# dpfried/action-segmentation

Measured on AMD Instinct MI355X. Metric: frames/sec semi-Markov decode, CrossTask T~10k K~20 L=1024, 1/2/4/8 GPUs, higher is better.
Workload: dtype f64

## Files before the change

### action-segmentation_amd/csrc/smm_api.hip

```cpp
#include <algorithm>
#include <atomic>
#include <functional>
#include <cstdio>
#include <cstdlib>
#include <cstring>
#include <numeric>
#include <vector>
#include <unordered_map>
#include <mutex>
#include <utility>
#include <string>

#include "../../include/smmdp.h"
#include "smm_device.h"
#include "smm_launch.h"
#include "smm_plan_feedback.h"

static thread_local int g_last_hip = 0;

namespace {
struct SmmEnv {
    int spec = 1;
    int no_split = 0;
    double split_min_us = 100.0, split_ns = 0.0;
// ... 225 lines not shown
    for (int i = 0; i < s->b; ++i)
        if (lengths[i] < 1 || lengths[i] > s->t_max) return false;
    return true;
}

struct Carver {
    size_t cur;
    size_t packed(size_t bytes) { const size_t o = cur; cur += bytes; return o; }
    size_t take(size_t bytes) { const size_t o = packed(bytes); cur = align_up(cur, 256); return o; }
};

static void plan_meta(const smm_shape *s, SmmPlan *p)
{
    Carver c{0};
    c.take(sizeof(SmmVideo) * s->b);
    p->o_order = c.take(sizeof(int32_t) * s->b);
    p->o_nstates = c.take(sizeof(int32_t) * s->n_groups);
    p->o_emcum = c.take(sizeof(int32_t) * ((size_t)s->b + 1));
    p->o_err = c.cur;
    p->meta_bytes = p->o_err + 512;
}

static SmmPlan make_plan(const smm_shape *s, const int64_t *lengths)
{
    SmmPlan p{};
    p.b = (size_t)s->b;
    plan_meta(s, &p);
    size_t h = 0;
    for (int i = 0; i < s->b; ++i) h += 8 * (size_t)s->c_max * (size_t)(lengths[i] + 1);
    p.hist_doubles = h;
    p.elp_doubles = (size_t)s->total_frames * s->c_max;
    p.tab_doubles = (size_t)s->n_groups * s->c_max * ((size_t)s->c_max + 1 + s->k_rows) + (size_t)s->b * s->c_max;
    p.band_doubles = (size_t)s->n_groups * s->c_max * ((size_t)SMM_BAND_ROW + SMM_BAND_TAB + 64);
    {
        const size_t um = chunk_units_max(s);
        p.chunk_bytes = align_up(sizeof(int32_t) * s->b, 256) + align_up(sizeof(double) * um * s->c_max, 256) +
                        chunk_ext_meta_bytes(s->b, um, s->b);
    }
    p.o_chunk = align_up(p.meta_bytes + 8 * (p.hist_doubles + p.elp_doubles + p.tab_doubles + p.band_doubles), 256);
    p.total = p.o_chunk + p.chunk_bytes + 1024;
    return p;
}

extern "C" size_t smm_workspace_bytes(const smm_shape *shape, const int64_t *lengths_host)
{
    if (!shape_ok(shape) || !lengths_host || !lengths_ok(shape, lengths_host)) return 0;
    return make_plan(shape, lengths_host).total;
}

extern "C" size_t smm_error_word_offset(const smm_shape *shape)
{
    if (!shape_ok(shape)) return 0;
    SmmPlan p{};
    plan_meta(shape, &p);
    return p.o_err;
}

struct Staged {
    SmmVideo *videos;
    int32_t *order;
    int32_t *n_states;
    int32_t *err;
    double *hist;
    double *elp;
    double *tabs;
    double *band;
    bool band_mode;
    int32_t *em_cum;
    std::vector<int32_t> em_cum_host;
    int em_tpw, em_blocks;
    int kp_max, c_need;
    int n_split;
    SmmVideo *uvideos;
    int32_t *uorder, *porder;
    SmmChunkVideo *cvs;
    int32_t *redo;
    double *anchors;
    int n_cv, n_units, u_part1;
    int small_first, small_count;
    uint64_t *stamps = nullptr;
    hipEvent_t done = nullptr;
    void *fb_entry = nullptr;
    std::vector<int32_t> order_host, frames_host;
};

static bool band_mode(int kp_max, int c_need);

static int device_cus()
{
    static std::mutex mu;
    static int n_cu[64] = {};
    int dev = 0;
    if (hipGetDevice(&dev) != hipSuccess || dev < 0 || dev >= 64) return 0;
    std::lock_guard<std::mutex> lock(mu);
    if (!n_cu[dev] && hipDeviceGetAttribute(&n_cu[dev], hipDeviceAttributeMultiprocessorCount, dev) != hipSuccess) n_cu[dev] = 0;
    return n_cu[dev] > 0 ? n_cu[dev] : 0;
}

constexpr double SMM_BAND_NS_BASE = 145.0, SMM_BAND_NS_PER_STATE = 2.0;
extern "C" double smm_band_frame_ns(int n_states)
{
    if (n_states < 1 || n_states > SMM_MAX_STATES) return 0.0;
    return SMM_BAND_NS_BASE + SMM_BAND_NS_PER_STATE * n_states;
}

static double dp_frame_ns(bool band, int c) { return band ? smm_band_frame_ns(c) : 150.0 + 3.0 * c; }

static int choose_split(const SmmVideo *hv, int32_t *order, int b, int d, int c_max, int64_t total_frames)
{
    const SmmEnv &ev = env();
    if (b < 24 || ev.no_split) return 0;
    const int n_cu = device_cus();
    if (n_cu <= 0) return 0;
    const double em_us = (double)total_frames * (4.0 * d + 8.0 * c_max) / 4.0e6;
    if (em_us < ev.split_min_us) return 0;
    int tmax = 0;
    for (int i = 0; i < b; ++i) tmax = std::max(tmax, hv[i].T);
    const double split_ns = ev.split_ns > 0.0 ? ev.split_ns : 1.75 * smm_band_frame_ns(std::min(c_max, (int)SMM_MAX_STATES));
    const int thr = tmax - (int)(em_us * 1000.0 / split_ns) - ev.split_margin;
    int n1 = 0;
    for (int i = 0; i < b; ++i) n1 += hv[i].T >= thr;
    if (thr <= 0 || n1 < 1 || n1 > b / 3 || n1 > n_cu / 2 || b - n1 < 16 || b > 2 * n_cu) return 0;
    std::stable_partition(order, order + b, [&](int32_t v) { return hv[v].T >= thr; });
    return n1;
}

namespace {
struct PlanFeedback {
    uint64_t *stamps = nullptr;
    hipEvent_t done = nullptr;
    bool pending = false;
    bool have = false;
    bool busy = false;
    int evals_left = 5, n_replans = 0;
    int b = 0, n1_first = 0;
    double em_us = 0.0, end_before_us = 0.0, end_after_us = 0.0;
    std::vector<uint64_t> snap, used;
    std::vector<int32_t> order, frames;
};
constexpr int SMM_FEEDBACK_MAX_REPLANS = 4;
constexpr double SMM_FEEDBACK_MIN_GAIN = 0.02;
struct PlanEntry {
    PlanFeedback *fb = nullptr;
    std::vector<char> key;
    int device = 0;
    char *dev_meta = nullptr;
    SmmPlan plan{};
    Staged st{};
    hipEvent_t ready = nullptr;
    hipStream_t stream = nullptr;
    bool settled = false;
};
struct PlanSlabs {
    char *cur = nullptr;
    size_t left = 0;
    std::vector<std::pair<char *, size_t>> all;
};
struct PlanCache {
    std::mutex mu;
    std::unordered_map<uint64_t, std::vector<PlanEntry *>> entries;
    std::unordered_map<uint64_t, uint32_t> seen_once;
    size_t n = 0, bytes = 0, key_bytes = 0;
    size_t pinned_bytes = 0;
    uint64_t generation = 1;
    PlanSlabs slabs[64];
} g_plans;
// ... 11 lines not shown
    if (dev < 0 || dev >= 64) return nullptr;
    PlanSlabs &sl = g_plans.slabs[dev];
    bytes = align_up(bytes, 256);
    if (bytes > sl.left) {
        const size_t want = std::max(bytes, SMM_PLAN_SLAB);
        char *p = nullptr;
        if (hipMalloc(reinterpret_cast<void **>(&p), want) != hipSuccess) { (void)hipGetLastError(); return nullptr; }
        sl.all.emplace_back(p, want);
        sl.cur = p;
        sl.left = want;
    }
    char *r = sl.cur;
    sl.cur += bytes;
    sl.left -= bytes;
    return r;
}

void plan_key_append(std::vector<char> &k, const void *p, size_t n)
{
    const char *c = static_cast<const char *>(p);
    k.insert(k.end(), c, c + n);
}

std::vector<char> plan_key(const smm_shape *s, const int64_t *lengths, const int64_t *frame_off, const int32_t *group,
                           const int32_t *kp, const int32_t *n_states, bool for_viterbi, int cum_chunk, bool want_split)
{
    std::vector<char> k;
    k.reserve(sizeof(*s) + (size_t)s->b * 24 + (size_t)s->n_groups * 4 + 128);
    plan_key_append(k, s, sizeof(*s));
    plan_key_append(k, lengths, sizeof(int64_t) * s->b);
    plan_key_append(k, frame_off, sizeof(int64_t) * s->b);
    const char has[2] = {(char)(group != nullptr), (char)(kp != nullptr)};
    plan_key_append(k, has, 2);
    if (group) plan_key_append(k, group, sizeof(int32_t) * s->b);
    if (kp) plan_key_append(k, kp, sizeof(int32_t) * s->b);
    plan_key_append(k, n_states, sizeof(int32_t) * s->n_groups);
    const int32_t f[3] = {for_viterbi, cum_chunk, want_split};
    plan_key_append(k, f, sizeof(f));
    const std::string &ek = env().key;
    plan_key_append(k, ek.data(), ek.size() + 1);
    return k;
}

void feedback_arm(PlanEntry *e, Staged *out)
{
    PlanFeedback *fb = e->fb;
    if (!fb || !env().plan_feedback) return;
    out->fb_entry = e;
    if (fb->pending) {
        if (hipEventQuery(fb->done) != hipSuccess) { (void)hipGetLastError(); return; }
        fb->pending = false;
        bool complete = !fb->have && !fb->busy;
        for (int i = 0; complete && i < fb->b; ++i) complete = fb->stamps[2 * i] > 0 && fb->stamps[2 * i + 1] >= fb->stamps[2 * i];
        if (complete) { fb->snap.assign(fb->stamps, fb->stamps + 2 * (size_t)fb->b); fb->have = true; }
    }
    if (fb->evals_left > 0 && !fb->have && !fb->busy) {
        std::memset(fb->stamps, 0, sizeof(uint64_t) * 2 * (size_t)fb->b);
        out->stamps = fb->stamps;
        out->done = fb->done;
        fb->pending = true;
    }
}

void plan_point(const SmmPlan &p, void *ws, Staged *out)
{
    char *base = static_cast<char *>(ws);
    out->err = reinterpret_cast<int32_t *>(base + p.o_err);
    out->hist = reinterpret_cast<double *>(base + p.meta_bytes);
    out->elp = out->hist + p.hist_doubles;
    out->tabs = out->elp + p.elp_doubles;
    out->band = out->tabs + p.tab_doubles;
    out->redo = reinterpret_cast<int32_t *>(base + p.o_chunk);
    out->anchors = reinterpret_cast<double *>(base + p.o_chunk + align_up(sizeof(int32_t) * p.b, 256));
}
}

static int stage_uncached(const smm_shape *s, const int64_t *lengths, const int64_t *frame_off, const int32_t *group,
                          const int32_t *kp, const int32_t *n_states, void *ws, size_t ws_bytes, hipStream_t stream, Staged *out,
                          bool for_viterbi, int cum_chunk, bool want_split, const std::function<char *(size_t)> *meta_alloc,
                          SmmPlan *plan_out);

static int stage(const smm_shape *s, const int64_t *lengths, const int64_t *frame_off, const int32_t *group,
                 const int32_t *kp, const int32_t *n_states, void *ws, size_t ws_bytes, hipStream_t stream, Staged *out,
                 bool for_viterbi = false, int cum_chunk = 0, bool want_split = false)
{
    if (!shape_ok(s) || !lengths || !frame_off || !n_states || !ws) return SMM_ERR_ARG;
    if (!env().plan_cache) return stage_uncached(s, lengths, frame_off, group, kp, n_states, ws, ws_bytes, stream, out, for_viterbi, cum_chunk, want_split, nullptr, nullptr);
    int dev = 0;
    if (hipGetDevice(&dev) != hipSuccess) dev = 0;
    hipStreamCaptureStatus cap = hipStreamCaptureStatusNone;
    if (hipStreamIsCapturing(stream, &cap) != hipSuccess) cap = hipStreamCaptureStatusNone;
    const bool capturing = cap != hipStreamCaptureStatusNone;
    const std::vector<char> key = plan_key(s, lengths, frame_off, group, kp, n_states, for_viterbi, cum_chunk, want_split);
    const uint64_t hk = plan_hash(key) ^ (uint64_t)dev;
    PlanEntry *hit = nullptr;
    {
        std::lock_guard<std::mutex> lock(g_plans.mu);
        auto it = g_plans.entries.find(hk);
        if (it != g_plans.entries.end())
            for (PlanEntry *e : it->second)
                if (e->device == dev && e->key.size() == key.size() && std::memcmp(e->key.data(), key.data(), key.size()) == 0) { hit = e; break; }
        if (hit && !hit->settled) {
            if (capturing) { if (hit->stream != stream) hit = nullptr; }
            else if (hipEventQuery(hit->ready) == hipSuccess) hit->settled = true;
            else if (hit->stream != stream && hipStreamWaitEvent(stream, hit->ready, 0) != hipSuccess) hit = nullptr;
        }
    }
    if (hit) {
        if (ws_bytes < hit->plan.total) return SMM_ERR_WORKSPACE;
        {
            std::lock_guard<std::mutex> lock(g_plans.mu);
            *out = hit->st;
            if (!capturing && for_viterbi && want_split) feedback_arm(hit, out);
        }
        plan_point(hit->plan, ws, out);
        char *base = static_cast<char *>(ws);
        SMM_HIP((hipError_t)smm_zero_async(base + hit->plan.o_err, hit->plan.meta_bytes - hit->plan.o_err, stream));
        return SMM_OK;
    }
    char *dev_meta = nullptr;
    bool keep = !capturing;
    if (keep) {
        std::lock_guard<std::mutex> lock(g_plans.mu);
        auto seen = g_plans.seen_once.find(hk);
        if (seen == g_plans.seen_once.end()) {
            if (g_plans.seen_once.size() >= 4 * SMM_PLAN_MAX_ENTRIES) g_plans.seen_once.clear();
            g_plans.seen_once.emplace(hk, 1u);
            keep = false;
        }
    }
    const std::function<char *(size_t)> alloc = [&](size_t bytes) -> char * {
        std::lock_guard<std::mutex> lock(g_plans.mu);
        if (!(g_plans.bytes + bytes <= SMM_PLAN_MAX_BYTES && g_plans.n < SMM_PLAN_MAX_ENTRIES &&
              g_plans.key_bytes + key.size() <= SMM_PLAN_MAX_BYTES)) return nullptr;
        dev_meta = plan_alloc(bytes, dev);
        if (dev_meta) g_plans.bytes += align_up(bytes, 256);
        return dev_meta;
    };
    SmmPlan plan{};
    const int rc = stage_uncached(s, lengths, frame_off, group, kp, n_states, ws, ws_bytes, stream, out, for_viterbi, cum_chunk, want_split,
                                  keep ? &alloc : nullptr, &plan);
    keep = keep && dev_meta != nullptr;
    if (rc != SMM_OK || !keep) return rc;
    PlanEntry *e = new PlanEntry;
    e->key = key;
    e->device = dev;
    e->dev_meta = dev_meta;
    e->plan = plan;
    PlanFeedback *fb = nullptr;
    std::vector<int32_t> order_host = std::move(out->order_host), frames_host = std::move(out->frames_host);
    out->order_host.clear(); out->frames_host.clear();
    e->st = *out;
    e->stream = stream;
    if (for_viterbi && want_split && env().plan_feedback && out->n_split > 0 && out->n_cv == 0 && out->small_count == 0 &&
        (int)order_host.size() == s->b) {
        fb = new PlanFeedback;
        const size_t bytes = sizeof(uint64_t) * 2 * (size_t)s->b;
        if (hipHostMalloc(reinterpret_cast<void **>(&fb->stamps), bytes, hipHostMallocDefault) != hipSuccess) fb->stamps = nullptr;
        if (fb->stamps && hipEventCreateWithFlags(&fb->done, hipEventDisableTiming) != hipSuccess) fb->done = nullptr;
        if (!fb->stamps || !fb->done) {
            (void)hipGetLastError();
            if (fb->stamps) (void)hipHostFree(fb->stamps);
            delete fb;
            fb = nullptr;
        } else {
            fb->b = s->b;
            fb->n1_first = out->n_split;
            fb->em_us = (double)s->total_frames * (4.0 * s->d + 8.0 * s->c_max) / 4.0e6;
            fb->order = std::move(order_host);
            fb->frames = std::move(frames_host);
            std::memset(fb->stamps, 0, bytes);
            fb->pending = true;
            out->stamps = fb->stamps;
            out->done = fb->done;
        }
    }
    e->fb = fb;
    auto drop_fb = [&]() {
        if (!fb) return;
        out->stamps = nullptr; out->done = nullptr;
        (void)hipHostFree(fb->stamps);
        (void)hipEventDestroy(fb->done);
        delete fb;
    };
    if (hipEventCreateWithFlags(&e->ready, hipEventDisableTiming) != hipSuccess || hipEventRecord(e->ready, stream) != hipSuccess) {
        if (e->ready) (void)hipEventDestroy(e->ready);
        drop_fb();
        delete e;
        return SMM_OK;
    }
    std::lock_guard<std::mutex> lock(g_plans.mu);
    if (fb) { g_plans.pinned_bytes += sizeof(uint64_t) * 2 * (size_t)s->b; out->fb_entry = e; }
    g_plans.entries[hk].push_back(e);
    g_plans.seen_once.erase(hk);
    g_plans.n += 1;
    g_plans.key_bytes += key.size();
    return SMM_OK;
}

// ... 717 lines not shown
    hipStream_t hs = static_cast<hipStream_t>(stream);
    int rc = stage(shape, lengths_host, frame_offset_host, group_host, kp_host, n_states_host, workspace, workspace_bytes,
                   hs, &st, true);
    if (rc != SMM_OK) return rc;
    if (!elp || !trans || !init || !len_scores) return SMM_ERR_ARG;
    const size_t g = shape->n_groups, cm = shape->c_max;
    double *t64 = st.tabs, *i64 = t64 + g * cm * cm, *l64 = i64 + g * cm, *e64 = l64 + g * shape->k_rows * cm;
    smm_launch_widen(trans, t64, g * cm * cm, hs);
    smm_launch_widen(init, i64, g * cm, hs);
    smm_launch_widen(len_scores, l64, g * shape->k_rows * cm, hs);
    if (endpen) smm_launch_widen(endpen, e64, (size_t)shape->b * cm, hs);
    smm_launch_widen(elp, st.elp, (size_t)shape->total_frames * cm, hs);
    SMM_HIP(hipGetLastError());
    return run_viterbi(shape, st, st.elp, t64, i64, l64, endpen ? e64 : nullptr, class_map, spans, labels, best, n_segs, hs);
}

namespace {
struct AuxDev {
    hipStream_t stream = nullptr, stream1 = nullptr;
    std::vector<std::pair<hipEvent_t, hipEvent_t>> events;
};
std::mutex g_aux_mu;
AuxDev g_aux[64];

hipStream_t aux_stream_n(int dev, int which)
{
    std::lock_guard<std::mutex> lock(g_aux_mu);
    AuxDev &d = g_aux[dev];
    hipStream_t &st = which ? d.stream1 : d.stream;
    if (!st) {
        int least = 0, greatest = 0;
        (void)hipDeviceGetStreamPriorityRange(&least, &greatest);
        if (hipStreamCreateWithPriority(&st, hipStreamNonBlocking, least) != hipSuccess) st = nullptr;
    }
    return st;
}
hipStream_t aux_stream(int dev) { return aux_stream_n(dev, 0); }

bool aux_events_get(int dev, std::pair<hipEvent_t, hipEvent_t> &ev)
{
    {
        std::lock_guard<std::mutex> lock(g_aux_mu);
        AuxDev &d = g_aux[dev];
        if (!d.events.empty()) { ev = d.events.back(); d.events.pop_back(); return true; }
    }
    ev = {nullptr, nullptr};
    if (hipEventCreateWithFlags(&ev.first, hipEventDisableTiming) != hipSuccess) return false;
    if (hipEventCreateWithFlags(&ev.second, hipEventDisableTiming) != hipSuccess) { (void)hipEventDestroy(ev.first); return false; }
    return true;
}

void aux_events_put(int dev, const std::pair<hipEvent_t, hipEvent_t> &ev)
{
    std::lock_guard<std::mutex> lock(g_aux_mu);
    g_aux[dev].events.push_back(ev);
}
}

static void release_aux()
{
    std::lock_guard<std::mutex> lock(g_aux_mu);
    for (int d = 0; d < 64; ++d) {
        for (auto &ev : g_aux[d].events) { (void)hipEventDestroy(ev.first); (void)hipEventDestroy(ev.second); }
        g_aux[d].events.clear();
        if (g_aux[d].stream) { (void)hipStreamDestroy(g_aux[d].stream); g_aux[d].stream = nullptr; }
        if (g_aux[d].stream1) { (void)hipStreamDestroy(g_aux[d].stream1); g_aux[d].stream1 = nullptr; }
    }
    std::lock_guard<std::mutex> lock2(g_dp_timing.mu);
    for (auto &ev : g_dp_timing.pool) { (void)hipEventDestroy(ev.first); (void)hipEventDestroy(ev.second); }
    g_dp_timing.pool.clear();
}

extern "C" int smm_decode_f32(const smm_shape *shape, const int64_t *lengths_host, const int64_t *frame_offset_host,
                              const int32_t *group_host, const int32_t *kp_host, const int32_t *n_states_host,
                              const float *x, const double *w, const double *cst, const double *inv_var, const float *cons,
                              const double *trans, const double *init, const double *len_scores, const double *endpen,
                              const int64_t *class_map, int64_t *spans, int64_t *labels, double *best, int32_t *n_segs,
                              float *elp32, void *workspace, size_t workspace_bytes, void *stream)
{
    g_fb_info = FeedbackInfo{};
    Staged st;
    hipStream_t hs = static_cast<hipStream_t>(stream);
    int rc = stage(shape, lengths_host, frame_offset_host, group_host, kp_host, n_states_host, workspace, workspace_bytes,
                   hs, &st, true, 0, true);
    if (rc != SMM_OK) return rc;
    int dev = 0;
    hipStream_t aux = nullptr;
    if (st.n_split > 0 && hipGetDevice(&dev) == hipSuccess && dev >= 0 && dev < 64) {
        hipStreamCaptureStatus cap = hipStreamCaptureStatusNone;
        if (hipStreamIsCapturing(hs, &cap) == hipSuccess && cap == hipStreamCaptureStatusNone) aux = aux_stream(dev);
    }
    std::pair<hipEvent_t, hipEvent_t> fj{nullptr, nullptr};
    if (aux && !aux_events_get(dev, fj)) aux = nullptr;
    if (!aux) {
        rc = run_emission(shape, st, x, w, cst, inv_var, cons, st.elp, elp32, hs);
        if (rc != SMM_OK) return rc;
        rc = run_viterbi(shape, st, st.elp, trans, init, len_scores, endpen, class_map, spans, labels, best, n_segs, hs);
        if (st.stamps && hipEventRecord(st.done, hs) != hipSuccess) (void)hipGetLastError();
        return rc;
    }
    const int n1 = st.n_split, n2 = shape->b - st.n_split;
    rc = run_viterbi(shape, st, st.elp, trans, init, len_scores, endpen, class_map, spans, labels, best, n_segs, hs, 0, n1, true, false);
    if (rc != SMM_OK) { aux_events_put(dev, fj); return rc; }
    const hipEvent_t fork = fj.first, join = fj.second;
    int rc2 = SMM_OK;
    rc = run_emission(shape, st, x, w, cst, inv_var, cons, st.elp, elp32, hs, 0, n1);
    if (rc != SMM_OK) { aux_events_put(dev, fj); return rc; }
    if (hipEventRecord(fork, hs) != hipSuccess || hipStreamWaitEvent(aux, fork, 0) != hipSuccess) rc2 = SMM_ERR_HIP;
#ifdef SMM_DEV
    const int dbg_split = env().split_debug;
#else
    const int dbg_split = 0;
#endif
    if (rc2 == SMM_OK && !(dbg_split & 2)) rc2 = run_emission(shape, st, x, w, cst, inv_var, cons, st.elp, elp32, aux, n1, n2);
    if (rc2 == SMM_OK && !(dbg_split & 1))
        rc2 = run_viterbi(shape, st, st.elp, trans, init, len_scores, endpen, class_map, spans, labels, best, n_segs, aux, n1, n2, false, true, 2);
    rc = run_viterbi(shape, st, st.elp, trans, init, len_scores, endpen, class_map, spans, labels, best, n_segs, hs, 0, n1, false, true, 1);
    if (hipEventRecord(join, aux) != hipSuccess || hipStreamWaitEvent(hs, join, 0) != hipSuccess) rc2 = SMM_ERR_HIP;
    aux_events_put(dev, fj);
    if (st.stamps && hipEventRecord(st.done, hs) != hipSuccess) (void)hipGetLastError();
    if (rc == SMM_OK && rc2 == SMM_OK) feedback_evaluate(st, hs);
    return rc != SMM_OK ? rc : rc2;
}

extern "C" int smm_logz_f64(const smm_shape *shape, const int64_t *lengths_host, const int64_t *frame_offset_host,
                            const int32_t *group_host, const int32_t *kp_host, const int32_t *n_states_host,
                            const double *elp, const double *trans, const double *init, const double *len_scores,
                            const double *endpen, double *logz, void *workspace, size_t workspace_bytes, void *stream)
{
    Staged st;
    hipStream_t hs = static_cast<hipStream_t>(stream);
    int rc = stage(shape, lengths_host, frame_offset_host, group_host, kp_host, n_states_host, workspace, workspace_bytes,
                   hs, &st);
    if (rc != SMM_OK) return rc;
    if (!elp || !trans || !init || !len_scores || !logz) return SMM_ERR_ARG;
    SmmDpArgs a = dp_args(shape, st, Tables{elp, trans, init, len_scores, endpen, nullptr});
    if (shape->flags & SMM_SHAPE_LOGZ_BOTH) {
        const ReversedTabs rt = reversed_tabs(shape, st.tabs);
        smm_launch_transpose(trans, rt.trans_t, shape->n_groups, shape->c_max, hs);
        a.trans_t = rt.trans_t;
        a.logz_b = rt.logz_b;
        a.flags |= 64;
    }
    rc = smm_launch_logz(a, logz, ring_regs(st.kp_max), st.c_need, hs);
    if (rc != SMM_OK) return rc;
    SMM_HIP(hipGetLastError());
    return SMM_OK;
}

extern "C" int smm_logz_bwd_f64(const smm_shape *shape, const int64_t *lengths_host, const int64_t *frame_offset_host,
                                const int32_t *group_host, const int32_t *kp_host, const int32_t *n_states_host,
                                const double *elp, const double *trans, const double *init, const double *len_scores,
                                const double *endpen, const double *logz, const double *grad_logz, double *g_elp,
                                double *g_trans, double *g_init, double *g_len, void *workspace, size_t workspace_bytes,
                                void *stream)
{
    Staged st;
    hipStream_t hs = static_cast<hipStream_t>(stream);
    int rc = stage(shape, lengths_host, frame_offset_host, group_host, kp_host, n_states_host, workspace, workspace_bytes,
                   hs, &st);
    if (rc != SMM_OK) return rc;
    if (!elp || !trans || !init || !len_scores || !logz || !g_elp || !g_trans || !g_init || !g_len) return SMM_ERR_ARG;
    const size_t g = shape->n_groups, cm = shape->c_max;
    const bool no_eos = (shape->flags & SMM_SHAPE_NO_EOS) != 0;
    rc = run_reversed(shape, st, st.hist, st.tabs, Tables{elp, trans, init, len_scores, endpen, logz}, hs);
    if (rc != SMM_OK) return rc;
    {
        void *const zp[4] = {g_trans, g_init, g_len, g_elp};
        const size_t zb[4] = {sizeof(double) * g * cm * cm, sizeof(double) * g * cm, sizeof(double) * g * shape->k_rows * cm,
                              sizeof(double) * (size_t)shape->total_frames * cm};
        SMM_HIP((hipError_t)smm_zero_multi_async(zp, zb, 4, hs));
    }
    SmmBwdArgs m{st.videos, st.n_states, trans, len_scores, st.hist, logz, grad_logz, g_elp, g_trans, g_init, g_len,
                 shape->c_max, shape->k_rows, shape->b, elp, no_eos ? 1 : 0};
    smm_launch_marginals(m, shape->t_max, st.kp_max, hs);
    SMM_HIP(hipGetLastError());
    return SMM_OK;
}

extern "C" int smm_sample_f64(const smm_shape *shape, const int64_t *lengths_host, const int64_t *frame_offset_host,
                              const int32_t *group_host, const int32_t *kp_host, const int32_t *n_states_host,
                              const double *elp, const double *trans, const double *init, const double *len_scores,
                              const double *endpen, const int64_t *class_map, const double *logz, int32_t n_samples,
                              uint64_t seed, int64_t *spans_out, int64_t *labels_out, double *logp_out, void *workspace,
                              size_t workspace_bytes, void *stream)
{
    if (n_samples <= 0 || (!spans_out && !labels_out && !logp_out)) return SMM_ERR_ARG;
    Staged st;
    hipStream_t hs = static_cast<hipStream_t>(stream);
// ... 954 lines not shown
```

### action-segmentation_amd/csrc/smm_viterbi.hip

```cpp
#include <type_traits>
#include "smm_device.h"

#ifdef SMM_PROFILE
#define SMM_PROF_DECL unsigned long long p_busy = 0, p_wait = 0, p_t0 = __builtin_readcyclecounter(), p_ph[4] = {0, 0, 0, 0}, p_mx = 0
#define SMM_BLOCK_BARRIER()                                                        \
    do {                                                                          \
        const unsigned long long t1 = __builtin_readcyclecounter();               \
        __syncthreads();                                                          \
        const unsigned long long t2 = __builtin_readcyclecounter();               \
        p_busy += t1 - p_t0; p_wait += t2 - t1; p_t0 = t2;                        \
    } while (0)
#define SMM_LDS_BARRIER()                                                          \
    do {                                                                          \
        const unsigned long long t1 = __builtin_readcyclecounter();               \
        smm_lds_barrier();                                                        \
        const unsigned long long t2 = __builtin_readcyclecounter();               \
        p_busy += t1 - p_t0; p_wait += t2 - t1;                                   \
        if (SMM_PROFILE == 2) { if (t2 - t1 < 150) { p_mx += 1; p_ph[jj & 3] += 1; p_ph[0] += (t1 - p_t0) << 20; } } \
        else { p_ph[jj & 3] += t1 - p_t0; p_mx = (t1 - p_t0 > p_mx) ? t1 - p_t0 : p_mx; } \
        p_t0 = t2;                                                                \
    } while (0)
#define SMM_PROF_OUT()                                                            \
    if (blockIdx.x == 0 && lane == 0) {                                           \
        unsigned long long *pp = reinterpret_cast<unsigned long long *>(a.err);   \
        pp[8 + w] = p_busy; pp[24 + w] = p_wait; pp[7] = (unsigned long long)J;   \
        if (BAND) { pp[16 + w] = p_mx; for (int ph = 0; ph < 4; ++ph) pp[32 + 4 * w + ph] = p_ph[ph]; } \
    }
#else
#define SMM_PROF_DECL do { } while (0)
#define SMM_BLOCK_BARRIER() __syncthreads()
#define SMM_LDS_BARRIER() smm_lds_barrier()
#define SMM_PROF_OUT() do { } while (0)
#endif

__device__ __forceinline__ void smm_lds_barrier()
{
    asm volatile("s_waitcnt lgkmcnt(0)\n\ts_barrier" ::: "memory");
}

#ifndef SMM_B
#define SMM_B 4
#endif
#ifndef SMM_D
#define SMM_D 1
#endif
#ifndef SMM_MOVER_STATES
#define SMM_MOVER_STATES 0
#endif
#ifndef SMM_CHAIN_DUAL
#define SMM_CHAIN_DUAL 1
#endif
#ifndef SMM_ABLATE
#define SMM_ABLATE 0
#endif
#ifndef SMM_SPEC
#define SMM_SPEC 1
#endif
#ifndef SMM_PIPE0_ALWAYS
#define SMM_PIPE0_ALWAYS 0
#endif
#ifndef SMM_SPEC8
#define SMM_SPEC8 0
#endif
#ifndef SMM_DOM_SPARSE
#define SMM_DOM_SPARSE 3
#endif
#ifndef SMM_ANCHOR
#define SMM_ANCHOR 0
#endif
#ifndef SMM_BAND_ALLWIT
#define SMM_BAND_ALLWIT 1
#endif
#ifndef SMM_HQ_ALWAYS
#define SMM_HQ_ALWAYS 0
#endif
#ifndef SMM_B8_R
#define SMM_B8_R 4
#endif

__device__ __forceinline__ void smm_best3(double &v, int &k, int &c, double v2, int k2, int c2)
{
    bool take = (v2 > v) || (v2 == v && (k2 < k || (k2 == k && c2 < c)));
    if (take) { v = v2; k = k2; c = c2; }
}

__device__ __forceinline__ void smm_wave_best3(double &v, int &k, int &c)
{
#pragma unroll
    for (int off = 32; off >= 1; off >>= 1) {
        double v2 = __shfl_xor(v, off);
        int k2 = __shfl_xor(k, off);
        int c2 = __shfl_xor(c, off);
        smm_best3(v, k, c, v2, k2, c2);
    }
}

template <int R>
__device__ __forceinline__ void smm_push(double (&A)[R], double (&L)[R], double hs, int u)
{
#pragma unroll
    for (int r0 = 0; r0 < R; r0 += 4) {
        double tq[4];
#pragma unroll
        for (int q = 0; q < 4; ++q)
            if (r0 + q < R) tq[q] = hs + L[(r0 + q - u + R) % R];
#pragma unroll
        for (int q = 0; q < 4; ++q)
            if (r0 + q < R) A[r0 + q] = smm_fmax(A[r0 + q], tq[q]);
    }
    L[(2 * R - 1 - u) % R] = smm_wave_ror1(L[(2 * R - 1 - u) % R]);
}

template <int R, int B, int D, bool TRIB = false>
__device__ __forceinline__ void smm_ring_block(double (&A)[R], double (&L)[R], double &hd, const double *h_blk,
                                               double *a_blk, int j, int jj, int lane, const double &ninf)
{
    constexpr int RING = 64 * R;
    double hv[B];
#pragma unroll
    for (int i = 0; i < B; ++i) hv[i] = h_blk[i * 2 * SMM_GH_STRIDE];
    if constexpr (D == 1) {
        smm_push<R>(A, L, hd, (jj * B) % R);
#pragma unroll
        for (int i = 1; i < B; ++i) smm_push<R>(A, L, hv[i - 1], (jj * B + i) % R);
        hd = hv[B - 1];
    } else {
#pragma unroll
        for (int i = 0; i < B; ++i) smm_push<R>(A, L, hv[i], (jj * B + i) % R);
    }
    if constexpr (R % B == 0) {
        if (lane == (((j + 1) * B) & (RING - 1)) / R) {
#pragma unroll
            for (int i = 0; i < B; ++i) {
                const int r = ((jj + 1) * B + i) % R;
                a_blk[i * SMM_MAX_STATES_DEV] = A[r];
                A[r] = ninf;
            }
        }
    } else if constexpr (B % R == 0) {
        const int d = lane - (((j + 1) * B) & (RING - 1)) / R;
// ... 230 lines not shown
    if (w == MW) {
#pragma unroll
        for (int q = 0; q < NE; ++q) {
            const int e = lane + 64 * q;
            mv_lo[q] = (e < B * cm) ? (e / cm) * SMM_MAX_STATES_DEV + e % cm : -1;
            const int64_t eg = (int64_t)B * cm + e;
            mv_pre[q] = elp[eg < e_last ? eg : e_last];
        }
    }
    auto mover_step = [&](int j, int jj, bool prefetch) -> double {
        const int mc = lane & (SMM_MAX_STATES_DEV - 1), mh = lane >> 5;
        double ev[B];
        double2 gh[PB];
#pragma unroll
        for (int i = 0; i < B; ++i) ev[i] = sh_e[(jj + 1) & 1][i][mc];
#pragma unroll
        for (int i = 0; i < PB; ++i) gh[i] = *reinterpret_cast<const double2 *>(&sh_gh[(jj + 1) & 1][mh * PB + i][mc][0]);
        __builtin_amdgcn_sched_barrier(0);
        if (prefetch) {
            double *dst = &sh_e[(jj + 1) & 1][0][0];
#pragma unroll
            for (int q = 0; q < NE; ++q)
                if (mv_lo[q] >= 0) dst[mv_lo[q]] = mv_pre[q];
#pragma unroll
            for (int q = 0; q < NE; ++q) {
                const int64_t e = (int64_t)(j + 2) * B * cm + lane + 64 * q;
                mv_pre[q] = elp[e < e_last ? e : e_last];
            }
        }
        double cv[PB];
#pragma unroll
        for (int i = 0; i < B; ++i) {
            mv_cum = mv_cum + ev[i];
            if (i / PB == 0) { if (mh == 0) cv[i % PB] = mv_cum; }
            else { if (mh == 1) cv[i % PB] = mv_cum; }
        }
        double hmax = gh[0].y;
#pragma unroll
        for (int i = 1; i < PB; ++i) hmax = smm_fmax(hmax, gh[i].y);
        if (j >= 1 && mc < C) {
            const int n0 = (j - 1) * B + 1 + mh * PB;
            double *hrow = hh + (size_t)mc * (T + 1) + n0;
            if (n0 + PB - 1 <= T) {
#pragma unroll
                for (int i = 0; i < PB; ++i) {
                    hcum[(size_t)(n0 + i) * C + mc] = cv[i];
                    hgam[(size_t)(n0 + i) * C + mc] = gh[i].x;
                    hrow[i] = gh[i].y;
                }
            } else {
#pragma unroll
                for (int i = 0; i < PB; ++i) {
                    if (n0 + i <= T) {
                        hcum[(size_t)(n0 + i) * C + mc] = cv[i];
                        hgam[(size_t)(n0 + i) * C + mc] = gh[i].x;
                        hrow[i] = gh[i].y;
                    }
                }
            }
        }
        return smm_max_halves(hmax);
    };
    if (w == 0) {
        __builtin_amdgcn_s_setprio(3);
        auto chain = [&](auto hf_c) {
            constexpr int HFC = decltype(hf_c)::value;
            constexpr int LG = (HFC == 4) ? 16 : 32;
            const int to = lane & (LG - 1), half = lane / LG;
            const bool live = to < C;
            double tr[HFC];
    #pragma unroll
            for (int i = 0; i < HFC; ++i) {
                const int f = half * HFC + i;
                tr[i] = (live && f < C) ? trans[(size_t)to * cm + f] : SMM_NEG_INF;
            }
            double lk[K0 + 1];
    #pragma unroll
            for (int k = 1; k <= K0; ++k) lk[k] = (live && k <= kp - 1) ? len[(size_t)k * cm + to] : SMM_NEG_INF;
            double hq[M];
    #pragma unroll
            for (int i = 0; i < M; ++i) hq[i] = SMM_NEG_INF;
            hq[0] = live ? (chunk_flat ? 0.0 : init[to]) : SMM_NEG_INF;
            double cum = (chunk_flat && live) ? anchor[to] : 0.0;
            double *const st_gam = half ? &sh_junk[0][0][to][0] : &sh_gam[to];
            double *const st_gh = half ? &sh_junk[0][0][to][0] : &sh_gh[0][0][to][0];
            constexpr int UC = M / B;
            SMM_PROF_DECL;
#ifdef SMM_PROFILE
            unsigned long long p_fastn = 0;
#endif
            bool spec = false;
            int cs = 0, spec_wait = 0, spec_back = 1;
            int sb_wait = 0, sb_back = 1;
#ifdef SMM_PROFILE
            unsigned long long p_sb_ok = 0, p_sb_fail = 0;
#endif
            double trS = SMM_NEG_INF, dlt = SMM_NEG_INF;
            const bool spec_off = !SPEC || (a.flags & 256);
            if (spec_off) spec_wait = 0x7fffffff;
            __builtin_amdgcn_s_waitcnt(0x0F70);
            for (int j0 = 0; j0 < J; j0 += UC) {
    #pragma unroll
                for (int jj = 0; jj < UC; ++jj) {
                    const int j = j0 + jj;
                    if (j >= J) break;
                    constexpr bool TIGHT = SPEC && B == 8 && HFC != 4;
                    double ap[B], ev[B];
                    auto stage = [&](int i) {
                        if (i < B) { ap[i] = sh_apart[jj & 1][i][to]; ev[i] = sh_e[jj & 1][i][to]; }
                    };
                    auto partial = [&](int i) {
                        double acc = ap[i];
                        if constexpr (SMM_ABLATE & 1) return acc;
                        const int kmax = TRI ? B + D + i : K0;
    #pragma unroll
                        for (int k0 = K0; k0 >= 2; k0 -= 4) {
                            double sq[4];
    #pragma unroll
                            for (int q = 0; q < 4; ++q)
                                if (k0 - q >= 2 && k0 - q <= kmax) sq[q] = hq[(jj * B + 1 + i - (k0 - q) + 4 * M) % M] + lk[k0 - q];
    #pragma unroll
                            for (int q = 0; q < 4; ++q)
                                if (k0 - q >= 2 && k0 - q <= kmax) acc = smm_fmax(acc, sq[q]);
                            if constexpr (TIGHT) { if (k0 - 4 >= 2) __builtin_amdgcn_sched_barrier(0); }
                        }
                        return acc;
                    };
                    bool block_done = false;
                    if constexpr (SPEC && SMM_SPEC8) {
                        if (spec && sb_wait == 0) {
                            double cumv[B], pp[B];
                            {
                                double apv[B], evv[B];
    #pragma unroll
                                for (int i = 0; i < B; ++i) { apv[i] = sh_apart[jj & 1][i][to]; evv[i] = sh_e[jj & 1][i][to]; }
    #pragma unroll
                                for (int i = 0; i < B; ++i) {
                                    double acc = SMM_NEG_INF;
                                    const int kmax = TRI ? B + D + i : K0;
    #pragma unroll
                                    for (int k0 = K0; k0 >= 1; k0 -= 4) {
                                        double sq[4];
    #pragma unroll
                                        for (int q = 0; q < 4; ++q)
                                            if (k0 - q > i && k0 - q <= kmax) sq[q] = hq[(jj * B + 1 + i - (k0 - q) + 4 * M) % M] + lk[k0 - q];
    #pragma unroll
                                        for (int q = 0; q < 4; ++q)
                                            if (k0 - q > i && k0 - q <= kmax) acc = smm_fmax(acc, sq[q]);
                                    }
                                    pp[i] = acc;
                                }
                                __builtin_amdgcn_sched_barrier(0);
                                double cr = cum;
    #pragma unroll
                                for (int i = 0; i < B; ++i) {
                                    cr = cr + evv[i];
                                    cumv[i] = cr;
                                    pp[i] = smm_fmax(pp[i], apv[i]);
                                }
                            }
                            double gsv[B], hg[B];
    #pragma unroll
                            for (int i = 0; i < B; ++i) gsv[i] = smm_readlane(cumv[i] + pp[i], cs);
    #pragma unroll
                            for (int i = 0; i < B; ++i) hg[i] = (gsv[i] + trS) - cumv[i];
                            double viol = SMM_NEG_INF;
    #pragma unroll
                            for (int i = 0; i < B; ++i) {
                                double acc = pp[i];
                                const int kmax = TRI ? B + D + i : K0;
    #pragma unroll
                                for (int k = 1; k <= i; ++k)
                                    if (k <= kmax) acc = smm_fmax(acc, hg[i - k] + lk[k]);
                                const double gm = cumv[i] + acc;
                                viol = smm_fmax(viol, gm - gsv[i]);
                                *reinterpret_cast<double2 *>(st_gh + ((jj & 1) * B + i) * 2 * SMM_GH_STRIDE) = make_double2(gm, hg[i]);
                            }
                            if (__ballot(viol > dlt) == 0) {
    #pragma unroll
                                for (int i = 0; i < B; ++i) hq[(jj * B + 1 + i) % M] = hg[i];
                                cum = cumv[B - 1];
                                block_done = true;
                                sb_back = 1;
#ifdef SMM_PROFILE
                                p_fastn += B; ++p_sb_ok;
#endif
                            } else {
                                sb_wait = sb_back;
                                sb_back = sb_back < 8 ? 2 * sb_back : 8;
#ifdef SMM_PROFILE
                                ++p_sb_fail;
#endif
                            }
                        } else if (sb_wait > 0) {
                            --sb_wait;
                        }
                    }
                    if (!block_done) {
                    if constexpr (TIGHT) { stage(0); stage(1); stage(2); }
                    else {
    #pragma unroll
                        for (int i = 0; i < B; ++i) stage(i);
                    }
                    double pacc = partial(0);
                    double cumn = (SMM_ABLATE & 2) ? ev[0] : cum + ev[0];
                    const bool spec0 = spec;
                    double gm_last = SMM_NEG_INF;
                    auto fold_read = [&](int i, double2 (&gv)[HFC / 2]) {
                        (void)i;
                        const double2 *gp = reinterpret_cast<const double2 *>(&sh_gam[half * HFC]);
    #pragma unroll
                        for (int q = 0; q < HFC / 2; ++q) gv[q] = gp[(SMM_ABLATE & 16) ? q % 2 : q];
                    };
                    auto fold_reduce = [&](const double2 (&gv)[HFC / 2]) {
                        double bq[4];
    #pragma unroll
                        for (int q = 0; q < ((SMM_ABLATE & 16) ? 2 : HFC / 2); ++q) {
                            if (q < 2) {
                                bq[2 * q] = gv[q].x + tr[2 * q];
                                bq[2 * q + 1] = gv[q].y + tr[2 * q + 1];
                            } else {
                                bq[(2 * q) & 3] = smm_fmax(bq[(2 * q) & 3], gv[q].x + tr[2 * q]);
                                bq[(2 * q + 1) & 3] = smm_fmax(bq[(2 * q + 1) & 3], gv[q].y + tr[2 * q + 1]);
                            }
                        }
                        double bm = smm_fmax(smm_fmax(bq[0], bq[1]), smm_fmax(bq[2], bq[3]));
                        if constexpr (HFC == 4) bm = smm_max_rows16(bm);
                        return smm_max_halves(bm);
                    };
                    constexpr bool PIPE0 = !TIGHT || SMM_PIPE0_ALWAYS;
                    auto run_block = [&](auto mode_c) {
                        constexpr int MODE = decltype(mode_c)::value;
    #pragma unroll
                        for (int i = 0; i < B; ++i) {
                            if constexpr (TIGHT) stage(i + 3);
                            const double acc = smm_fmax(pacc, hq[(jj * B + i + 4 * M) % M] + lk[1]);
                            cum = cumn;
                            const double gm = cum + acc;
                            {
                                double hcur;
                                if constexpr (MODE == 1) {
                                    const double gs = (SMM_ABLATE & 512) ? dlt : smm_readlane(gm, cs);
                                    const bool bad = (SMM_ABLATE & 512) ? spec_wait == 12345 : __ballot(gm - gs > dlt) != 0;
                                    const double hfast = (gs + trS) - cum;
                                    __builtin_amdgcn_sched_barrier(0);
                                    if (i + 1 < B) {
                                        pacc = partial(i + 1 < B ? i + 1 : 0);
                                        cumn = cum + ev[i + 1 < B ? i + 1 : 0];
                                    }
                                    __builtin_amdgcn_sched_barrier(0);
                                    asm volatile("" : "+v"(pacc), "+v"(cumn));
                                    double hfast_p = hfast;
                                    asm volatile("" : "+v"(hfast_p));
                                    if (__builtin_expect(bad, 0)) {
                                        st_gam[0] = gm;
                                        const double2 *gp = reinterpret_cast<const double2 *>(&sh_gam[half * HFC]);
                                        double bm = SMM_NEG_INF;
    #pragma unroll
                                        for (int q = 0; q < HFC / 2; ++q) {
                                            const double2 g2 = gp[q];
                                            bm = smm_fmax(bm, smm_fmax(g2.x + tr[2 * q], g2.y + tr[2 * q + 1]));
                                            __builtin_amdgcn_sched_barrier(0);
                                        }
                                        if constexpr (HFC == 4) bm = smm_max_rows16(bm);
                                        hcur = smm_max_halves(bm) - cum;
                                        if (spec) { spec = false; dlt = SMM_NEG_INF; }
                                        if (i == B - 1) gm_last = gm;
                                    } else {
                                        hcur = hfast_p;
#ifdef SMM_PROFILE
                                        ++p_fastn;
#endif
                                    }
                                } else {
                                    double2 gv[HFC / 2];
                                    st_gam[0] = gm;
                                    fold_read(i, gv);
                                    __builtin_amdgcn_sched_barrier(0);
                                    if constexpr (PIPE0) {
                                        if (i + 1 < B) {
                                            pacc = partial(i + 1 < B ? i + 1 : 0);
                                            cumn = (SMM_ABLATE & 2) ? ev[i + 1 < B ? i + 1 : 0] : cum + ev[i + 1 < B ? i + 1 : 0];
                                        }
                                        __builtin_amdgcn_sched_barrier(0);
                                    }
                                    hcur = fold_reduce(gv) - cum;
                                    if constexpr (!PIPE0) {
                                        __builtin_amdgcn_sched_barrier(0);
                                        if (i + 1 < B) {
                                            pacc = partial(i + 1 < B ? i + 1 : 0);
                                            cumn = cum + ev[i + 1 < B ? i + 1 : 0];
                                        }
                                    }
                                    if (i == B - 1) gm_last = gm;
                                }
                                hq[(jj * B + 1 + i) % M] = hcur;
                                *reinterpret_cast<double2 *>(st_gh + ((jj & 1) * B + i) * 2 * SMM_GH_STRIDE) = make_double2(gm, hcur);
                            }
                        }
                    };
                    if (SPEC && spec) run_block(std::integral_constant<int, SPEC ? 1 : 0>{});
                    else run_block(std::integral_constant<int, 0>{});
                    if constexpr (SPEC) {
                        if (spec0 && !spec) { spec_wait = 0; spec_back = 1; }
                        if (!spec && --spec_wait < 0) {
                            const double v = (live && half == 0) ? gm_last : SMM_NEG_INF;
                            const double rmax = smm_row_max16(v);
                            const double best = fmax(smm_readlane(rmax, 0), smm_readlane(rmax, 16));
                            const unsigned long long lead_m = __ballot(v == best && live && half == 0);
                            bool ok = false;
                            if (lead_m) {
                                cs = __builtin_amdgcn_readfirstlane(__ffsll(lead_m) - 1);
                                int to_i = to < SN ? to : 0;
                                asm volatile("" : "+v"(to_i));
                                trS = sh_tr[to_i * SN + cs];
                                dlt = sh_dl[cs * SN + to_i];
                                ok = __ballot(gm_last - best > dlt) == 0;
                            }
                            if (ok) { spec = true; spec_back = 1; }
                            else { dlt = SMM_NEG_INF; spec_wait = spec_back; spec_back = spec_back < 32 ? 2 * spec_back : 32; }
                        }
                    }
                    }
                    SMM_LDS_BARRIER();
                }
            }
            if (half == 0) sh_gfin[to] = sh_gh[(J - 1) & 1][(T - 1) % B][to][0];
#ifdef SMM_PROFILE
            p_ph[2] = p_fastn;
            p_ph[1] = p_sb_ok; p_ph[3] = p_sb_fail;
#endif
            SMM_PROF_OUT();
        };
        if constexpr (BAND && HF > 4 && SMM_CHAIN_DUAL) {
            if (C <= 16) chain(std::integral_constant<int, 4>{});
            else chain(std::integral_constant<int, HF>{});
        } else {
            chain(std::integral_constant<int, HF>{});
        }
    } else if (BAND) {
      if constexpr (BAND) {
        constexpr int SPS = SPW, RS = 2, NBD = SMM_BAND_N;
        static_assert(!BAND || SPS * NBD <= 64, "one lane per (state, band) of a pusher wave");
        constexpr int NPS = NP - 1;
        const int rank = (w == MW) ? (1 << 20) : ((w < MW) ? w - 1 : w - 2);
        const double *lent = a.len_t + (size_t)g * cm * SMM_BAND_ROW;
        const double *btab = a.band_tab + (size_t)g * cm * SMM_BAND_TAB;
        const bool bound_ok = kp - 1 >= 32 + 15 + 127;
        double As[SPS][RS];
        constexpr int NHR = (SPS * B + 15) / 16;
        constexpr int BPG = 16 / B;
        constexpr int UBB = UB;
        static_assert(!BAND || (UB == BPG && K0 < SMM_BAND_LO), "a group is one unrolled iteration of the block loop");
        static_assert(!BAND || D == 0, "DOM: the block's own sources, all of them in the rows read at its start");
        int hoff[NHR];
        double xdom[NHR];
#pragma unroll
        for (int r = 0; r < NHR; ++r) {
            const int e = 16 * r + (lane & 15), ejs = e / B, ec = ejs * NPS + rank;
            hoff[r] = ((e % B) * SMM_GH_STRIDE + ((ejs < SPS && ec < C) ? ec : 0)) * 2 + 1;
            xdom[r] = sh_xd[BAND ? ((ejs < SPS && ec < C) ? ec : 0) : 0];
        }
        constexpr bool ANCHOR = SMM_ANCHOR != 0;
        static_assert(!BAND || !ANCHOR || (TRI ? B + D + 1 : 2 * B + D) >= 9, "dlow covers band 0's lengths from 9 on (smm_band_tables_kernel)");
        double anc_h[SPS];
        int anc_s[SPS];
#pragma unroll
        for (int js = 0; js < SPS; ++js) {
            const int ec = js * NPS + rank;
            anc_h[js] = (BAND && ec < C) ? init[ec] : SMM_NEG_INF;
            anc_s[js] = 0;
        }
        const int dlim = ANCHOR ? kp - 1 - 127 : 0;
        uint32_t nanch = 0;
        uint32_t npush = 0;
        unsigned long long mcur = 0, mnext = 0;
        const int nvw = (rank < C) ? ((C - 1 - rank) / NPS + 1 < SPS ? (C - 1 - rank) / NPS + 1 : SPS) : 0;
        uint32_t nact = 0;
#pragma unroll
        for (int js = 0; js < SPS; ++js) {
#pragma unroll
            for (int r = 0; r < RS; ++r) As[js][r] = SMM_NEG_INF;
        }
        static_assert(!BAND || BPG == 2, "a group is two blocks: decided in the second block of the previous group");
        static_assert(!BAND || (SMM_BAND_DELAY - 2 * B) / B - 1 >= 4 + 4, "delayed-band reads of the history: at least 4 block steps of slack behind the mover's drained stores");
        double hmx = SMM_NEG_INF;
        const int qjs = lane >> 3, qm = (lane & 7) + 1;
        const int qc = qjs * NPS + rank;
        const bool qok = qjs < SPS && qc < C && SMM_BAND_LO + SMM_BAND_DELAY * qm <= kp - 1;
        const double *qcol = hh + (size_t)((qjs < SPS && qc < C) ? qc : 0) * (T + 1);
        const double qlmx = qok ? btab[(size_t)qc * SMM_BAND_TAB + qm] : SMM_NEG_INF;
        const double qlbm = (qok && bound_ok) ? btab[(size_t)qc * SMM_BAND_TAB] : SMM_NEG_INF;
        const double *qhm = &sh_hm[BAND ? ((qjs < SPS && qc < C) ? qc : 0) : 0][0];
        constexpr int NWIT = 7;
        double qmlw[NWIT];
#pragma unroll
        for (int t = 0; t < NWIT; ++t) {
            const int dlt = 7 * (qm - 1) + 2 + t;
            qmlw[t] = (qjs < SPS && qc < C && dlt <= SMM_BAND_WIT && 16 * dlt + 142 <= kp - 1) ? btab[(size_t)qc * SMM_BAND_TAB + 16 + dlt] : SMM_NEG_INF;
        }
        double hq[2][B];
#pragma unroll
        for (int i = 0; i < B; ++i) { hq[0][i] = SMM_NEG_INF; hq[1][i] = SMM_NEG_INF; }
        constexpr int NPRE = 2;
        double Lp[NPRE][RS];
// ... 656 lines not shown
```

Baseline: 999.6 million.

## Defer workspace zeroing to side stream and precompute next-step partial in chain

The host side defers the metadata zero-fill on plan-cache hits and, when splitting, issues that zero-fill and the first Viterbi part on the aux stream, joined back with events, so they overlap with emission on the main stream. In the Viterbi chain kernel with B==8, the partial max over older history for the next block step is computed at the end of the current step, before the LDS barrier, instead of at the start of the next step. This takes it off the critical path after the barrier. The cost is extra events and stream synchronization, and a loop-carried register value.

```diff
diff --git a/action-segmentation_amd/csrc/smm_api.hip b/action-segmentation_amd/csrc/smm_api.hip
--- a/action-segmentation_amd/csrc/smm_api.hip
+++ b/action-segmentation_amd/csrc/smm_api.hip
@@ -331,6 +331,8 @@
     hipEvent_t done = nullptr;
     void *fb_entry = nullptr;
     std::vector<int32_t> order_host, frames_host;
+    void *zero_ptr = nullptr;
+    size_t zero_bytes = 0;
 };
 
 static bool band_mode(int kp_max, int c_need);
@@ -508,7 +510,7 @@
 
 static int stage(const smm_shape *s, const int64_t *lengths, const int64_t *frame_off, const int32_t *group,
                  const int32_t *kp, const int32_t *n_states, void *ws, size_t ws_bytes, hipStream_t stream, Staged *out,
-                 bool for_viterbi = false, int cum_chunk = 0, bool want_split = false)
+                 bool for_viterbi = false, int cum_chunk = 0, bool want_split = false, bool defer_zero = false)
 {
     if (!shape_ok(s) || !lengths || !frame_off || !n_states || !ws) return SMM_ERR_ARG;
     if (!env().plan_cache) return stage_uncached(s, lengths, frame_off, group, kp, n_states, ws, ws_bytes, stream, out, for_viterbi, cum_chunk, want_split, nullptr, nullptr);
@@ -541,6 +543,11 @@
         }
         plan_point(hit->plan, ws, out);
         char *base = static_cast<char *>(ws);
+        if (defer_zero && !capturing) {
+            out->zero_ptr = base + hit->plan.o_err;
+            out->zero_bytes = hit->plan.meta_bytes - hit->plan.o_err;
+            return SMM_OK;
+        }
         SMM_HIP((hipError_t)smm_zero_async(base + hit->plan.o_err, hit->plan.meta_bytes - hit->plan.o_err, stream));
         return SMM_OK;
     }
@@ -1424,7 +1431,7 @@
     Staged st;
     hipStream_t hs = static_cast<hipStream_t>(stream);
     int rc = stage(shape, lengths_host, frame_offset_host, group_host, kp_host, n_states_host, workspace, workspace_bytes,
-                   hs, &st, true, 0, true);
+                   hs, &st, true, 0, true, true);
     if (rc != SMM_OK) return rc;
     int dev = 0;
     hipStream_t aux = nullptr;
@@ -1435,6 +1442,7 @@
     std::pair<hipEvent_t, hipEvent_t> fj{nullptr, nullptr};
     if (aux && !aux_events_get(dev, fj)) aux = nullptr;
     if (!aux) {
+        if (st.zero_bytes) SMM_HIP((hipError_t)smm_zero_async(st.zero_ptr, st.zero_bytes, hs));
         rc = run_emission(shape, st, x, w, cst, inv_var, cons, st.elp, elp32, hs);
         if (rc != SMM_OK) return rc;
         rc = run_viterbi(shape, st, st.elp, trans, init, len_scores, endpen, class_map, spans, labels, best, n_segs, hs);
@@ -1442,11 +1450,20 @@
         return rc;
     }
     const int n1 = st.n_split, n2 = shape->b - st.n_split;
-    rc = run_viterbi(shape, st, st.elp, trans, init, len_scores, endpen, class_map, spans, labels, best, n_segs, hs, 0, n1, true, false);
-    if (rc != SMM_OK) { aux_events_put(dev, fj); return rc; }
+    std::pair<hipEvent_t, hipEvent_t> pj{nullptr, nullptr};
+    bool side_prep = aux_events_get(dev, pj);
+    if (side_prep && hipEventRecord(pj.first, hs) != hipSuccess) { (void)hipGetLastError(); side_prep = false; }
     const hipEvent_t fork = fj.first, join = fj.second;
     int rc2 = SMM_OK;
     rc = run_emission(shape, st, x, w, cst, inv_var, cons, st.elp, elp32, hs, 0, n1);
+    if (side_prep && hipStreamWaitEvent(aux, pj.first, 0) != hipSuccess) { (void)hipGetLastError(); side_prep = false; }
+    const hipStream_t ps = side_prep ? aux : hs;
+    if (rc == SMM_OK && st.zero_bytes && smm_zero_async(st.zero_ptr, st.zero_bytes, ps) != (int)hipSuccess) rc = SMM_ERR_HIP;
+    if (rc == SMM_OK)
+        rc = run_viterbi(shape, st, st.elp, trans, init, len_scores, endpen, class_map, spans, labels, best, n_segs, ps, 0, n1, true, false);
+    if (side_prep && (hipEventRecord(pj.second, aux) != hipSuccess || hipStreamWaitEvent(hs, pj.second, 0) != hipSuccess) && rc == SMM_OK)
+        rc = SMM_ERR_HIP;
+    if (pj.first) aux_events_put(dev, pj);
     if (rc != SMM_OK) { aux_events_put(dev, fj); return rc; }
     if (hipEventRecord(fork, hs) != hipSuccess || hipStreamWaitEvent(aux, fork, 0) != hipSuccess) rc2 = SMM_ERR_HIP;
 #ifdef SMM_DEV
diff --git a/action-segmentation_amd/csrc/smm_viterbi.hip b/action-segmentation_amd/csrc/smm_viterbi.hip
--- a/action-segmentation_amd/csrc/smm_viterbi.hip
+++ b/action-segmentation_amd/csrc/smm_viterbi.hip
@@ -56,6 +56,9 @@
 #ifndef SMM_SPEC
 #define SMM_SPEC 1
 #endif
+#ifndef SMM_CHAIN_PRE
+#define SMM_CHAIN_PRE 1
+#endif
 #ifndef SMM_PIPE0_ALWAYS
 #define SMM_PIPE0_ALWAYS 0
 #endif
@@ -452,6 +455,8 @@
             for (int i = 0; i < M; ++i) hq[i] = SMM_NEG_INF;
             hq[0] = live ? (chunk_flat ? 0.0 : init[to]) : SMM_NEG_INF;
             double cum = (chunk_flat && live) ? anchor[to] : 0.0;
+            constexpr bool PRE = SMM_CHAIN_PRE != 0 && B == 8;
+            double pnext = SMM_NEG_INF;
             double *const st_gam = half ? &sh_junk[0][0][to][0] : &sh_gam[to];
             double *const st_gh = half ? &sh_junk[0][0][to][0] : &sh_gh[0][0][to][0];
             constexpr int UC = M / B;
@@ -572,7 +577,7 @@
     #pragma unroll
                         for (int i = 0; i < B; ++i) stage(i);
                     }
-                    double pacc = partial(0);
+                    double pacc = PRE ? smm_fmax(ap[0], pnext) : partial(0);
                     double cumn = (SMM_ABLATE & 2) ? ev[0] : cum + ev[0];
                     const bool spec0 = spec;
                     double gm_last = SMM_NEG_INF;
@@ -691,6 +696,25 @@
                             else { dlt = SMM_NEG_INF; spec_wait = spec_back; spec_back = spec_back < 32 ? 2 * spec_back : 32; }
                         }
                     }
+                    }
+                    if constexpr (PRE) {
+                        constexpr int kmax = TRI ? B + D : K0;
+                        bool have = false;
+    #pragma unroll
+                        for (int k0 = K0; k0 >= 2; k0 -= 4) {
+                            double sq[4];
+    #pragma unroll
+                            for (int q = 0; q < 4; ++q)
+                                if (k0 - q >= 2 && k0 - q <= kmax) sq[q] = hq[((jj + 1) * B + 1 - (k0 - q) + 4 * M) % M] + lk[k0 - q];
+    #pragma unroll
+                            for (int q = 0; q < 4; ++q)
+                                if (k0 - q >= 2 && k0 - q <= kmax) {
+                                    pnext = have ? smm_fmax(pnext, sq[q]) : sq[q];
+                                    have = true;
+                                }
+                            if constexpr (TIGHT) { if (k0 - 4 >= 2) __builtin_amdgcn_sched_barrier(0); }
+                        }
+                        asm volatile("" : "+v"(pnext));
                     }
                     SMM_LDS_BARRIER();
                 }
```

After: 997.9 million, median of 2. No clear change (-0.2%).
